# bliunlpr/Robust_e2e_gan

Measured on AMD Instinct MI355X. Metric: joint_train utterances/sec, higher is better.
Workload: dtype f32; 1 GPU; config4: joint_train.py full GAN+ASR step, B=32 per GPU, T=800, F=257->80, L=40, V=4233, enhancer 2xBLSTM-256, VGG+3xBLSTMP-512, loc-attention decoder 300, D basic ndf64, Adadelta; global_batch=32, per_rank_batch=32, parallelism=dp1, utterance_lengths=560..800 frames (mean 680 of T=800)

## Files before the change

### robust_e2e_gan_amd/csrc/lstm.hip

```cpp
#include <stdlib.h>

#include <atomic>

#include "common.h"

namespace {

#ifdef RE2E_EXPERIMENTS
__device__ unsigned long long* g_lstm_stamps = nullptr;
constexpr int kStampStep0 = 64;
#define LSTM_STAMP_DECL unsigned long long* const stamp_p = g_lstm_stamps
#define LSTM_STAMP(ph)                                                                                                              \
  do {                                                                                                                              \
    if (stamp_p && (threadIdx.x & 63) == 0 && s >= kStampStep0 && s < kStampStep0 + 16)                                             \
      stamp_p[((((long)blockIdx.z * gridDim.y + blockIdx.y) * gridDim.x + blockIdx.x) * 16 + (threadIdx.x >> 6)) * 192 + (s - kStampStep0) * 12 + (ph)] = \
          (ph) >= 10 ? __builtin_amdgcn_s_memrealtime() : __builtin_amdgcn_s_memtime();                                             \
  } while (0)
static void lstm_stamps_arm() {
  const char* v = getenv("RE2E_LSTM_STAMPS");
  unsigned long long* p = v ? (unsigned long long*)strtoull(v, nullptr, 16) : nullptr;
  (void)hipMemcpyToSymbol(HIP_SYMBOL(g_lstm_stamps), &p, sizeof(p));
}
#else
#define LSTM_STAMP_DECL
// ... 95 lines not shown
    int idx = tid + it * NTH;
    int bm = idx >> 3, jj = idx & 7, b = b0 + bm, j = j0 + jj;
    if (idx >= 256 || b >= B) continue;
    float v[4];
#pragma unroll
    for (int g = 0; g < 4; ++g) {
      float a = 0.f;
      for (int w = 0; w < WAVES; ++w) a += red[w * (32 * 33) + bm * 33 + g * 8 + jj];
      v[g] = a + pre[it][g];
    }
    float gi = sigmoidf_(v[0]), gf = sigmoidf_(v[1]), gg = tanhf_(v[2]), go = sigmoidf_(v[3]);
    float c = gf * cp[it] + gi * gg;
    float h = go * tanhf_(c);
    if (t >= ln[it]) { c = 0.f; h = 0.f; }
    float* go_ = xg + ((long)t * B + b) * 4 * H + j;
    go_[0] = gi; go_[H] = gf; go_[2 * H] = gg; go_[3 * H] = go;
    cbuf[((long)(t + 1) * B + b) * H2 + dir * H + j] = c;
    ybuf[((long)(t + 1) * B + b) * H2 + dir * H + j] = h;
    hf_wr[((long)(j >> 2) * 32 + bm) * 4 + (j & 3)] = h;
  }
}

typedef unsigned long long u64;
typedef unsigned u32x4 __attribute__((ext_vector_type(4)));
typedef __attribute__((address_space(1))) u64 gu64;
__device__ unsigned g_persist_aborts = 0;
constexpr unsigned kSpinLimit = 1u << 24;

template <int WAVES, int QN, int UW>
__global__ __launch_bounds__(WAVES * 64) void lstm_fwd_persist(float* xg_f, float* xg_r, const float* __restrict__ wfrag, float* ybuf,
                                                               float* cbuf, u64* hx_, unsigned* err, const int* __restrict__ lens,
                                                               int T, int B, int H) {
  extern __shared__ __attribute__((aligned(16))) float red[];
  static_assert(WAVES >= 4 * UW, "256 threads per 8 units own the 32 x 8 cell updates");
  const int dir = blockIdx.z, mt = blockIdx.y, MT = gridDim.y, NX = gridDim.x * UW;
  const int tid = threadIdx.x, lane = tid & 63, wid = tid >> 6, lr = lane & 31, lh = lane >> 5;
  const int usub = (tid >> 8) < UW ? (tid >> 8) : 0;
  const int x = blockIdx.x * UW + usub;
  float* xg = dir ? xg_r : xg_f;
  const int j0 = x * 8, b0 = mt * 32;
  constexpr int kAbort = UW * WAVES * 32 * 33;
  if (tid == 0) red[kAbort] = 0.f;
  const long H2 = 2L * H;
  f32x4 w[UW][QN];
#pragma unroll
  for (int u = 0; u < UW; ++u) {
    const f32x4* wp = reinterpret_cast<const f32x4*>(wfrag) + ((long)(dir * NX + blockIdx.x * UW + u) * NX + wid * QN) * 64 + lane;
#pragma unroll
    for (int q = 0; q < QN; ++q) w[u][q] = wp[q * 64];
  }
  gu64* hx = (gu64*)hx_;
  const int par_sz = 2 * MT * NX * 256;
  const __amdgpu_buffer_rsrc_t hx_rs = __builtin_amdgcn_make_buffer_rsrc(hx_, 0, (int)(2 * par_sz * 8), 0x00020000);
  const int grp = (dir * MT + mt) * NX * 256;
  const int rd_off = grp + (wid * QN) * 256 + (lh * 32 + lr) * 4;
  const bool pw = tid < 256 * UW;
  const int bm = (tid >> 3) & 31, jj = tid & 7, b = b0 + bm, j = j0 + jj;
  const bool ok = pw && b < B;
  const int ln = ok ? lens[b] : 0;
  const int wr_off = grp + x * 256 + ((jj >> 2) * 32 + bm) * 4 + (jj & 3);
  float c = 0.f, pre[4] = {0.f, 0.f, 0.f, 0.f};
  if (ok) {
    const float* gp = xg + ((long)(dir ? T - 1 : 0) * B + b) * 4 * H + j;
#pragma unroll
    for (int g = 0; g < 4; ++g) pre[g] = gp[g * H];
  }
  LSTM_STAMP_DECL;
  __syncthreads();
  for (int s = 0; s < T; ++s) {
    const int t = dir ? T - 1 - s : s;
    LSTM_STAMP(0); LSTM_STAMP(10);
    f32x16 acc[UW];
// ... 1 lines not shown
    for (int u = 0; u < UW; ++u)
#pragma unroll
      for (int r = 0; r < 16; ++r) acc[u][r] = 0.f;
    if (s > 0) {
      const gu64* src = hx + ((s & 1) ^ 1) * par_sz + rd_off;
      float hv[QN][4];
      const unsigned rd_b = (unsigned)((((s & 1) ^ 1) * par_sz + rd_off) * 8);
      for (unsigned spins = 0;; ++spins) {
        asm volatile("" ::: "memory");
        bool good = true;
#pragma unroll
        for (int q = 0; q < QN; ++q) {
          const u32x4 lo = __builtin_amdgcn_raw_buffer_load_b128(hx_rs, rd_b + (unsigned)q * 2048u, 0, 16);
          const u32x4 hi = __builtin_amdgcn_raw_buffer_load_b128(hx_rs, rd_b + (unsigned)q * 2048u + 16u, 0, 16);
          hv[q][0] = __uint_as_float(lo[0]); hv[q][1] = __uint_as_float(lo[2]);
          hv[q][2] = __uint_as_float(hi[0]); hv[q][3] = __uint_as_float(hi[2]);
          good &= (lo[1] == (unsigned)s) & (lo[3] == (unsigned)s) & (hi[1] == (unsigned)s) & (hi[3] == (unsigned)s);
        }
        if (__all(good)) break;
        if (spins > kSpinLimit) { if (lane == 0) { red[kAbort] = 1.f; if (atomicExch(err, 1u) == 0u) atomicAdd(&g_persist_aborts, 1u); } break; }
        __builtin_amdgcn_s_sleep(1);
      }
      LSTM_STAMP(1);
#pragma unroll
      for (int q = 0; q < QN; ++q)
#pragma unroll
        for (int i = 0; i < 4; ++i)
#pragma unroll
          for (int u = 0; u < UW; ++u) acc[u] = __builtin_amdgcn_mfma_f32_32x32x2f32(hv[q][i], w[u][q][i], acc[u], 0, 0, 0);
    }
#pragma unroll
    for (int u = 0; u < UW; ++u) store_acc(red + (u * WAVES + wid) * (32 * 33), acc[u], lane);
    LSTM_STAMP(2);
    __syncthreads();
    LSTM_STAMP(3);
    if (red[kAbort] != 0.f) break;
    if (pw) {
      float v[4];
#pragma unroll
      for (int g = 0; g < 4; ++g) {
        float a = 0.f;
#pragma unroll
        for (int wv = 0; wv < WAVES; ++wv) a += red[(usub * WAVES + wv) * (32 * 33) + bm * 33 + g * 8 + jj];
        v[g] = a + pre[g];
      }
      float gi = sigmoidf_(v[0]), gf = sigmoidf_(v[1]), gg = tanhf_(v[2]), go = sigmoidf_(v[3]);
      float cn = gf * c + gi * gg;
      float h = go * tanhf_(cn);
      if (t >= ln) { cn = 0.f; h = 0.f; }
      c = cn;
      if (ok && s + 1 < T) {
        const float* gp = xg + ((long)(dir ? t - 1 : t + 1) * B + b) * 4 * H + j;
// ... 8 lines not shown
        float* go_ = xg + ((long)t * B + b) * 4 * H + j;
        go_[0] = gi; go_[H] = gf; go_[2 * H] = gg; go_[3 * H] = go;
        cbuf[((long)(t + 1) * B + b) * H2 + dir * H + j] = cn;
        ybuf[((long)(t + 1) * B + b) * H2 + dir * H + j] = h;
      }
    }
    LSTM_STAMP(5);
    __syncthreads();
    LSTM_STAMP(6);
  }
  if (red[kAbort] != 0.f && ok) {
    for (int t = 0; t < T; ++t) ybuf[((long)(t + 1) * B + b) * H2 + dir * H + j] = __uint_as_float(0x7fc00000u);
  }
}

__device__ __forceinline__ void store16u_sc1(unsigned* p, const u32x4& v) {
  asm volatile("global_store_dwordx4 %0, %1, off sc1\n\ts_nop 1" ::"v"(p), "v"(v) : "memory");
}
constexpr unsigned kTagBit = 0x40000000u, kNanPub = 0x3FC00000u;
__device__ __forceinline__ bool tags_are(const u32x4& v, unsigned want) {
  return (((v[0] & v[1] & v[2] & v[3]) ^ want) & kTagBit) == 0u && (((v[0] | v[1] | v[2] | v[3]) ^ want) & kTagBit) == 0u;
}

template <int TILES, int NJ, bool PERSIST>
__global__ __launch_bounds__(256) void lstm_fwd2(float* xg_f, float* xg_r, const float* __restrict__ whh_f, const float* __restrict__ whh_r,
                                                 float* ybuf, float* cbuf, unsigned* hx_, unsigned* err, const int* __restrict__ lens, int T,
                                                 int B, int H, int s_arg) {
  constexpr int KS = 4;
  extern __shared__ __attribute__((aligned(16))) float lds2[];
  f32x4* part = reinterpret_cast<f32x4*>(lds2);
  int* abortw = reinterpret_cast<int*>(lds2 + 2 * TILES * KS * 64 * 4);
  const int dir = blockIdx.z, mt = blockIdx.y, MT = gridDim.y, x = blockIdx.x;
  const int tid = threadIdx.x, lane = tid & 63, ks = tid >> 6, n = lane & 15, kk = lane >> 4;
  const int ft = ks < TILES ? ks : -1;
  float* xg = dir ? xg_r : xg_f;
  const float* whh = dir ? whh_r : whh_f;
  const long H2 = 2L * H;
  if (PERSIST && tid == 0) *abortw = 0;
  f32x4 w[TILES][NJ];
#pragma unroll
  for (int t = 0; t < TILES; ++t) {
    const long row = (long)(n & 3) * H + 4 * TILES * x + 4 * t + (n >> 2);
#pragma unroll
    for (int jj = 0; jj < NJ; ++jj) w[t][jj] = *reinterpret_cast<const f32x4*>(whh + row * H + 16 * (ks * NJ + jj) + 4 * kk);
  }
  const int par_w = 2 * MT * H * 16;
  const __amdgpu_buffer_rsrc_t hx_rs = __builtin_amdgcn_make_buffer_rsrc(hx_, 0, (int)(2 * par_w * 4), 0x00020000);
  const bool fin = ft >= 0;
  const int j = 4 * TILES * x + 4 * (fin ? ft : 0) + kk;
  const int s0 = PERSIST ? 0 : s_arg, s1 = PERSIST ? T : s_arg + 1;
  const int grp = (dir * MT + mt) * H * 16;
  const int b = 16 * mt + n;
  const unsigned rd_w = (unsigned)(grp + ((4 * ks * NJ + kk) * 16 + n) * 4);
  const unsigned poll_w = (unsigned)(grp + ((4 * ks * NJ + (lane < 4 * NJ ? lane : 0)) * 16) * 4);
  const bool ok = fin && b < B;
  const int ln = ok ? lens[b] : 0;
  const unsigned wr_w = (unsigned)(grp + ((TILES * x + (fin ? ft : 0)) * 16 + n) * 4);
  float c = 0.f, pre[4] = {0.f, 0.f, 0.f, 0.f};
  if (ok) {
    const int t0 = dir ? T - 1 - s0 : s0;
    const float* gp = xg + ((long)t0 * B + b) * 4 * H + j;
#pragma unroll
    for (int g = 0; g < 4; ++g) pre[g] = gp[g * H];
    if (!PERSIST) c = cbuf[((long)(dir ? t0 + 2 : t0) * B + b) * H2 + dir * H + j];
  }
  u32x4 ld[NJ];
#pragma unroll
// ... 11 lines not shown
    constexpr int NACC = TILES == 1 ? 2 : TILES;
    f32x4 acc[NACC];
#pragma unroll
    for (int tt = 0; tt < NACC; ++tt) acc[tt] = f32x4{0.f, 0.f, 0.f, 0.f};
    if (s > 0) {
      const unsigned want = PERSIST ? (unsigned)((((s - 1) >> 1) + 1) & 1) << 30 : 0u;
      const unsigned rd_b = (unsigned)((((s & 1) ^ 1) * par_w) * 4) + rd_w * 4u;
      const unsigned pl_b = (unsigned)((((s & 1) ^ 1) * par_w) * 4) + poll_w * 4u;
      auto wait_producers = [&]() {
        for (unsigned spins = 0;; ++spins) {
          asm volatile("" ::: "memory");
          const u32x4 pv = __builtin_amdgcn_raw_buffer_load_b128(hx_rs, pl_b, 0, 16);
          if (__all(tags_are(pv, want))) break;
          if (spins > kSpinLimit) { if (lane == 0) { *abortw = 1; if (atomicExch(err, 1u) == 0u) atomicAdd(&g_persist_aborts, 1u); } break; }
        }
        asm volatile("" ::: "memory");
      };
      if (PERSIST) {
        wait_producers();
#pragma unroll
        for (int jj = 0; jj < NJ; ++jj) ld[jj] = __builtin_amdgcn_raw_buffer_load_b128(hx_rs, rd_b + (unsigned)jj * 1024u, 0, 16);
        LSTM_STAMP(7);
      }
#pragma unroll
      for (int jj = 0; jj < NJ; ++jj) {
        u32x4 v = ld[jj];
        if (PERSIST) {
          if (!__all(tags_are(v, want))) {
            wait_producers();
#pragma unroll
            for (int j2 = jj; j2 < NJ; ++j2) ld[j2] = __builtin_amdgcn_raw_buffer_load_b128(hx_rs, rd_b + (unsigned)j2 * 1024u, 0, 16);
            v = ld[jj];
            for (unsigned spins = 0; !__all(tags_are(v, want)); ++spins) {
              asm volatile("" ::: "memory");
              v = __builtin_amdgcn_raw_buffer_load_b128(hx_rs, rd_b + (unsigned)jj * 1024u, 0, 16);
              if (spins > kSpinLimit) { if (lane == 0) { *abortw = 1; if (atomicExch(err, 1u) == 0u) atomicAdd(&g_persist_aborts, 1u); } break; }
            }
          }
        }
        float hv[4];
#pragma unroll
        for (int i = 0; i < 4; ++i) {
          unsigned uu = PERSIST ? (v[i] & ~kTagBit) : v[i];
          if (PERSIST) uu = uu == kNanPub ? 0x7fc00000u : uu;
          hv[i] = __uint_as_float(uu);
        }
#pragma unroll
        for (int i = 0; i < 4; ++i)
#pragma unroll
          for (int tt = 0; tt < TILES; ++tt) {
            const int a = TILES == 1 ? (i & 1) : tt;
            acc[a] = __builtin_amdgcn_mfma_f32_16x16x4f32(w[tt][jj][i], hv[i], acc[a], 0, 0, 0);
          }
      }
      if (TILES == 1) acc[0] += acc[1];
    }
    LSTM_STAMP(1);
    f32x4* pp = part + (s & 1) * (TILES * KS * 64);
#pragma unroll
    for (int tt = 0; tt < TILES; ++tt)
      if (tt != ft) pp[(tt * KS + ks) * 64 + lane] = acc[tt];
    LSTM_STAMP(2);
    __syncthreads();
    LSTM_STAMP(3);
    if (PERSIST && *abortw) break;
    float og[6] = {0.f, 0.f, 0.f, 0.f, 0.f, 0.f};
    if (fin) {
      f32x4 v = {0.f, 0.f, 0.f, 0.f};
      f32x4 mine = acc[0];
#pragma unroll
      for (int tt = 1; tt < TILES; ++tt) mine = ft == tt ? acc[tt] : mine;
#pragma unroll
      for (int k2 = 0; k2 < KS; ++k2) v += k2 == ks ? mine : pp[(ft * KS + k2) * 64 + lane];
      const float gi = sigmoidf_(v[0] + pre[0]), gf = sigmoidf_(v[1] + pre[1]), gg = tanhf_(v[2] + pre[2]), go = sigmoidf_(v[3] + pre[3]);
      float cn = __builtin_fmaf(gf, c, gi * gg);
      float h = go * tanhf_(cn);
// ... 316 lines not shown
    LSTM_STAMP(8); LSTM_STAMP(11);
    if (lane == 0)
      __hip_atomic_store(flags + (s & 1) * f_par + f_grp + (long)x * 32 + wid * 8, (unsigned)(s + 1), __ATOMIC_RELAXED, __HIP_MEMORY_SCOPE_AGENT);
  }
#pragma unroll
  for (int u = 0; u < UW; ++u) {
    const int j = j0 + 8 * u + jj;
    if (ok) dc_state[(long)b * H2 + dir * H + j] = dcr[u];
    if (aborted && ok) {
      for (int t = 0; t < T; ++t) G[((long)t * B + b) * K4 + j] = __uint_as_float(0x7fc00000u);
    }
  }
}

__global__ void pack_w_bwd3_kernel(const float* __restrict__ whh, float* __restrict__ wb, int H, int UN) {
  const long tot = (long)(H / UN) * (H / 16) * UN * 64;
  for (long e = (long)blockIdx.x * blockDim.x + threadIdx.x; e < tot; e += (long)gridDim.x * blockDim.x) {
    const int lane = (int)(e & 63); long r = e >> 6; const int ks = (int)(r % UN); r /= UN; const int jt = (int)(r % (H / 16)); const int x = (int)(r / (H / 16));
    const int kappa = (lane >> 4) * UN + ks;
    wb[e] = whh[((long)(kappa / UN) * H + (long)x * UN + kappa % UN) * H + 16 * jt + (lane & 15)];
  }
}

template <int UN, int TPW>
__global__ __launch_bounds__(256) void lstm_bwd3(float* g_f, float* g_r, const float* __restrict__ wb, const float* __restrict__ dy,
                                                 const float* __restrict__ cbuf, float* dc_state, float* xbuf, unsigned* flags_, unsigned* err,
                                                 const int* __restrict__ lens, int T, int B, int H, float* __restrict__ dbp) {
  constexpr int KG = 4 * UN;
  constexpr int LDG = KG + 4;
  constexpr int BLK = 16 * UN;
  constexpr int BPI = 1024 / (BLK * 4);
  __shared__ __attribute__((aligned(16))) float dgs[16 * LDG];
  __shared__ __attribute__((aligned(16))) float psum[4 * 256];
  __shared__ int aborted;
  const int dir = blockIdx.z, mt = blockIdx.y, x = blockIdx.x, MT = gridDim.y, NX = gridDim.x;
  float* G = dir ? g_r : g_f;
  const int j0 = x * UN, b0 = mt * 16;
  const int tid = threadIdx.x, lane = tid & 63, wid = tid >> 6, n = lane & 15, kq = lane >> 4;
  const int K4 = 4 * H;
  const long H2 = 2L * H;
  if (tid == 0) aborted = 0;
  float wreg[TPW][UN];
  {
    const float* wp = wb + ((long)(dir * NX + x) * (H / 16)) * UN * 64 + lane;
#pragma unroll
    for (int u = 0; u < TPW; ++u)
#pragma unroll
      for (int ks = 0; ks < UN; ++ks) wreg[u][ks] = wp[((long)(wid + 4 * u) * UN + ks) * 64];
  }
  const long grp = (long)(dir * MT + mt);
  const long x_par = (long)2 * MT * NX * NX * BLK;
  float* xg = xbuf + grp * NX * NX * BLK;
  const __amdgpu_buffer_rsrc_t x_rs = __builtin_amdgcn_make_buffer_rsrc(xbuf, 0, (int)(2 * x_par * 4), 0x00020000);
  gu32* flags = (gu32*)flags_;
  const long f_par = (long)2 * MT * NX * 32;
  const long f_grp = grp * NX * 32;
  const bool cell = tid < 16 * UN;
  const int bm = cell ? tid / UN : 0, jj = tid % UN, b = b0 + bm, j = j0 + jj;
  const bool ok = cell && b < B;
  const long bb = ok ? b : 0;
  const int ln = lens[bb];
  float dcr = 0.f;
  float sbi = 0.f, sbf = 0.f, sbg = 0.f, sbo = 0.f;
  float n_dy, n_g[4], n_c, n_cp;
  {
    const int t = dir ? 0 : T - 1;
    const int prev_blk = dir ? t + 2 : t;
    n_dy = dy[((long)t * B + bb) * H2 + dir * H + j];
    const float* gp0 = G + ((long)t * B + bb) * K4 + j;
#pragma unroll
    for (int g = 0; g < 4; ++g) n_g[g] = gp0[g * H];
// ... 66 lines not shown
      if (cell) {
        const int e = bm * UN + jj;
        if (BPI == 1) dh += (psum[e] + psum[256 + e]) + (psum[512 + e] + psum[768 + e]);
        else dh += ((psum[e] + psum[128 + e]) + (psum[256 + e] + psum[384 + e])) + ((psum[512 + e] + psum[640 + e]) + (psum[768 + e] + psum[896 + e]));
      }
    }
    if (cell) {
      float di = 0.f, df = 0.f, dg = 0.f, dout = 0.f, dcp = dcr;
      if (ok && t < ln) {
        float tc = tanhf_(c);
        float dct = dh * go * (1.f - tc * tc) + dcr;
        dout = dh * tc * go * (1.f - go);
        di = dct * gg * gi * (1.f - gi);
        df = dct * cp * gf * (1.f - gf);
        dg = dct * gi * (1.f - gg * gg);
        dcp = dct * gf;
      }
      dcr = dcp;
      sbi += di; sbf += df; sbg += dg; sbo += dout;
      if (ok) {
        float* gp = G + ((long)t * B + b) * K4 + j;
        gp[0] = di; gp[H] = df; gp[2 * H] = dg; gp[3 * H] = dout;
      }
      float* dq = dgs + bm * LDG + jj;
      dq[0] = di; dq[UN] = df; dq[2 * UN] = dg; dq[3 * UN] = dout;
    }
    LSTM_STAMP(4);
    __syncthreads();
    LSTM_STAMP(5);
    if (s == T - 1) break;
    float bv[UN];
#pragma unroll
    for (int q = 0; q < UN / 4; ++q) {
      const f32x4 t4 = *reinterpret_cast<const f32x4*>(dgs + n * LDG + kq * UN + 4 * q);
      bv[4 * q] = t4[0]; bv[4 * q + 1] = t4[1]; bv[4 * q + 2] = t4[2]; bv[4 * q + 3] = t4[3];
    }
    float* xw = xg + (s & 1) * x_par;
    f32x4 acc[TPW];
    auto store_tile = [&](int u) {
      const int jc0 = 16 * (wid + 4 * u) + 4 * kq;
      float* dst = xw + ((long)(jc0 / UN) * NX + x) * BLK + n * UN + (jc0 % UN);
      store16_sc1(dst, acc[u]);
    };
#pragma unroll
    for (int u0 = 0; u0 < TPW; u0 += 2) {
      acc[u0] = f32x4{0.f, 0.f, 0.f, 0.f};
      if (u0 + 1 < TPW) acc[u0 + 1] = f32x4{0.f, 0.f, 0.f, 0.f};
#pragma unroll
      for (int ks = 0; ks < UN; ++ks) {
        acc[u0] = __builtin_amdgcn_mfma_f32_16x16x4f32(wreg[u0][ks], bv[ks], acc[u0], 0, 0, 0);
        if (u0 + 1 < TPW) acc[u0 + 1] = __builtin_amdgcn_mfma_f32_16x16x4f32(wreg[u0 + 1][ks], bv[ks], acc[u0 + 1], 0, 0, 0);
        if (u0 >= 2 && (ks == 1 || ks == 3)) {
          __builtin_amdgcn_sched_barrier(0);
          store_tile(u0 - 2 + (ks >> 1));
          __builtin_amdgcn_sched_barrier(0);
        }
      }
    }
    if (TPW % 2 == 0) store_tile(TPW - 2);
    store_tile(TPW - 1);
    LSTM_STAMP(6);
    asm volatile("s_waitcnt vmcnt(0)" ::: "memory");
    LSTM_STAMP(7); LSTM_STAMP(8); LSTM_STAMP(11);
    if (lane == 0)
      __hip_atomic_store(flags + (s & 1) * f_par + f_grp + (long)x * 32 + wid * 8, (unsigned)(s + 1), __ATOMIC_RELAXED, __HIP_MEMORY_SCOPE_AGENT);
  }
  if (ok) dc_state[(long)b * H2 + dir * H + j] = dcr;
  if (dbp) {
    __syncthreads();
    if (cell) {
      float* dq = dgs + bm * LDG + jj;
      dq[0] = sbi; dq[UN] = sbf; dq[2 * UN] = sbg; dq[3 * UN] = sbo;
    }
    __syncthreads();
// ... 78 lines not shown
bool is_built(SeqFamily family, int a, int b) {
#define RE2E_HAS(A, B) if (a == A && b == B) return true;
  switch (family) {
    case kFwd2Persist: case kFwd2Step: RE2E_FWD2_ALL(RE2E_HAS) break;
    case kFwdPersist: RE2E_FWD_PERSIST_ALL(RE2E_HAS) break;
    case kFwdStep: RE2E_FWD_STEP_ALL(RE2E_HAS) break;
    case kBwd3: RE2E_BWD3_ALL(RE2E_HAS) break;
    case kBwdPersist: RE2E_BWD_PERSIST_ALL(RE2E_HAS) break;
    case kBwdStep: RE2E_BWD_STEP_ALL(RE2E_HAS) break;
  }
#undef RE2E_HAS
  return false;
}

constexpr size_t kCuLds = 160 * 1024;
constexpr size_t kBwdStaticLds = 16 * 1024;
size_t own_cu_lds(long workgroups, int cus, size_t static_lds, size_t needed) {
  return workgroups <= cus / 2 ? kCuLds - static_lds : needed;
}

bool env_off(const char* name) {
  const char* v = getenv(name);
  return v && atoi(v) == 0;
}

bool plan_fwd(int T, int B, int H, bool weights_16B_aligned, int cus, SeqPlan& p) {
  if (H % 8 != 0) return false;
  const bool persist = !env_off("RE2E_LSTM_PERSIST") && T >= 2;
  if (!env_off("RE2E_LSTM_FWD2") && weights_16B_aligned && H % 64 == 0 && (B <= 16 || H >= 384)) {
    const long per = (long)cdiv(B, 16) * 2;
    int tiles = 0;
    for (int lim : {cus / 2, cus})
      for (int tl = 1; tl <= 4 && !tiles; tl *= 2)
        if ((long)(H / (4 * tl)) * per <= lim) tiles = tl;
    const bool resident = persist && tiles;
    if (!tiles) tiles = 4;
    if (is_built(kFwd2Persist, tiles, H / 64)) {
      p = {resident ? kFwd2Persist : kFwd2Step, tiles, H / 64, dim3(H / (4 * tiles), cdiv(B, 16), 2), (size_t)tiles * 8192 + 16};
      if (resident) p.lds = own_cu_lds((long)p.grid.x * p.grid.y * 2, cus, 0, p.lds);
      return true;
    }
  }
  const dim3 grid(H / 8, cdiv(B, 32), 2);
  if (persist && (long)grid.x * grid.y * 2 <= cus) {
#define RE2E_FIT(W, Q) if ((int)grid.x == W * Q) { p = {kFwdPersist, W, Q, grid, own_cu_lds((long)grid.x * grid.y * 2, cus, 0, (size_t)W * 32 * 33 * sizeof(float) + 16)}; return true; }
    RE2E_FWD_PERSIST_ALL(RE2E_FIT)
// ... 49 lines not shown
  float *wfrag, *hfrag;
  void* hxmem;
  size_t hxbytes;
};
struct BwdArgs {
  float *g_f, *g_r;
  const float *wb, *dy, *cbuf;
  float *dc, *slabs;
  const int* lens;
  int T, B, H;
  void* flagmem;
  size_t flagbytes;
  float* dbp;
};

template <int W>
void launch_fwd_step(const SeqPlan& p, const FwdArgs& a, hipStream_t st) {
  ensure_lds<&lstm_fwd_step<W>>(p.lds);
  const long hn = (long)2 * 2 * p.grid.y * a.H * 32;
  hipLaunchKernelGGL(zero_kernel, dim3(cdiv(hn, 256) > 1024 ? 1024 : cdiv(hn, 256)), dim3(256), 0, st, a.hfrag, hn);
  for (int s = 0; s < a.T; ++s)
    hipLaunchKernelGGL((lstm_fwd_step<W>), p.grid, dim3(W * 64), p.lds, st, a.xg_f, a.xg_r, a.wfrag, a.ybuf, a.cbuf, a.hfrag, a.lens, a.T, a.B, a.H, s);
}
template <int W, int QN>
void launch_fwd_persist(const SeqPlan& p, const FwdArgs& a, hipStream_t st) {
  ensure_lds<&lstm_fwd_persist<W, QN, 1>>(p.lds);
  lstm_stamps_arm();
  (void)hipMemsetAsync(a.hxmem, 0, a.hxbytes, st);
  hipLaunchKernelGGL((lstm_fwd_persist<W, QN, 1>), p.grid, dim3(W * 64), p.lds, st, a.xg_f, a.xg_r, a.wfrag, a.ybuf, a.cbuf, (u64*)((char*)a.hxmem + 16),
                     (unsigned*)a.hxmem, a.lens, a.T, a.B, a.H);
}
template <int TILES, int NJ>
void launch_fwd2_persist(const SeqPlan& p, const FwdArgs& a, hipStream_t st) {
  ensure_lds<&lstm_fwd2<TILES, NJ, true>>(p.lds);
  lstm_stamps_arm();
  (void)hipMemsetAsync(a.hxmem, 0, a.hxbytes, st);
  hipLaunchKernelGGL((lstm_fwd2<TILES, NJ, true>), p.grid, dim3(256), p.lds, st, a.xg_f, a.xg_r, a.whh_f, a.whh_r, a.ybuf, a.cbuf,
                     (unsigned*)((char*)a.hxmem + 16), (unsigned*)a.hxmem, a.lens, a.T, a.B, a.H, 0);
}
template <int TILES, int NJ>
void launch_fwd2_step(const SeqPlan& p, const FwdArgs& a, hipStream_t st) {
  ensure_lds<&lstm_fwd2<TILES, NJ, false>>(p.lds);
  for (int s = 0; s < a.T; ++s)
    hipLaunchKernelGGL((lstm_fwd2<TILES, NJ, false>), p.grid, dim3(256), p.lds, st, a.xg_f, a.xg_r, a.whh_f, a.whh_r, a.ybuf, a.cbuf,
                       (unsigned*)((char*)a.hxmem + 16), (unsigned*)a.hxmem, a.lens, a.T, a.B, a.H, s);
}
template <int JT>
void launch_bwd_step(const SeqPlan& p, const BwdArgs& a, hipStream_t st) {
  for (int s = 0; s < a.T; ++s)
    hipLaunchKernelGGL((lstm_bwd_step<JT>), p.grid, dim3(256), 0, st, a.g_f, a.g_r, a.wb, a.dy, a.cbuf, a.dc, a.slabs, a.lens, a.T, a.B, a.H, s);
}
template <int TPW, int UW>
void launch_bwd_persist(const SeqPlan& p, const BwdArgs& a, hipStream_t st) {
  lstm_stamps_arm();
  (void)hipMemsetAsync(a.flagmem, 0, a.flagbytes, st);
  ensure_lds<&lstm_bwd_persist<TPW, UW>>(p.lds);
  hipLaunchKernelGGL((lstm_bwd_persist<TPW, UW>), p.grid, dim3(256), p.lds, st, a.g_f, a.g_r, a.wb, a.dy, a.cbuf, a.dc, a.slabs,
                     (unsigned*)((char*)a.flagmem + 16), (unsigned*)a.flagmem, a.lens, a.T, a.B, a.H);
}
template <int UN, int TPW>
void launch_bwd3(const SeqPlan& p, const BwdArgs& a, hipStream_t st) {
  lstm_stamps_arm();
  (void)hipMemsetAsync(a.flagmem, 0, a.flagbytes, st);
  ensure_lds<&lstm_bwd3<UN, TPW>>(p.lds);
  hipLaunchKernelGGL((lstm_bwd3<UN, TPW>), p.grid, dim3(256), p.lds, st, a.g_f, a.g_r, a.wb, a.dy, a.cbuf, a.dc, a.slabs,
                     (unsigned*)((char*)a.flagmem + 16), (unsigned*)a.flagmem, a.lens, a.T, a.B, a.H, a.dbp);
}

int run_fwd(const SeqPlan& p, const FwdArgs& args, hipStream_t st) {
  switch (p.family) {
#define RE2E_F2P(A, B) if (p.a == A && p.b == B) return launch_fwd2_persist<A, B>(p, args, st), RE2E_OK;
#define RE2E_F2S(A, B) if (p.a == A && p.b == B) return launch_fwd2_step<A, B>(p, args, st), RE2E_OK;
#define RE2E_FP(A, B) if (p.a == A && p.b == B) return launch_fwd_persist<A, B>(p, args, st), RE2E_OK;
#define RE2E_FS(A, B) if (p.a == A) return launch_fwd_step<A>(p, args, st), RE2E_OK;
    case kFwd2Persist: RE2E_FWD2_ALL(RE2E_F2P) break;
    case kFwd2Step: RE2E_FWD2_ALL(RE2E_F2S) break;
    case kFwdPersist: RE2E_FWD_PERSIST_ALL(RE2E_FP) break;
    case kFwdStep: RE2E_FWD_STEP_ALL(RE2E_FS) break;
    default: break;
#undef RE2E_F2P
#undef RE2E_F2S
#undef RE2E_FP
#undef RE2E_FS
  }
  re2e_set_error("re2e_lstm_seq_fwd: plan %s(%d, %d) is not in the instantiation tables", kFamilyText[p.family].name, p.a, p.b);
  return RE2E_EUNSUPPORTED;
}
int run_bwd(const SeqPlan& p, const BwdArgs& args, hipStream_t st) {
  switch (p.family) {
#define RE2E_B3(A, B) if (p.a == A && p.b == B) return launch_bwd3<A, B>(p, args, st), RE2E_OK;
#define RE2E_BP(A, B) if (p.a == A && p.b == B) return launch_bwd_persist<A, B>(p, args, st), RE2E_OK;
#define RE2E_BS(A, B) if (p.a == A) return launch_bwd_step<A>(p, args, st), RE2E_OK;
    case kBwd3: RE2E_BWD3_ALL(RE2E_B3) break;
    case kBwdPersist: RE2E_BWD_PERSIST_ALL(RE2E_BP) break;
    case kBwdStep: RE2E_BWD_STEP_ALL(RE2E_BS) break;
    default: break;
#undef RE2E_B3
#undef RE2E_BP
#undef RE2E_BS
  }
  re2e_set_error("re2e_lstm_seq_bwd: plan %s(%d, %d) is not in the instantiation tables", kFamilyText[p.family].name, p.a, p.b);
  return RE2E_EUNSUPPORTED;
}

}

namespace {
std::atomic<int> g_force_abort{0};
bool debug_hooks_enabled() {
  static const bool on = [] { const char* e = getenv("RE2E_DEBUG_HOOKS"); return e && atoi(e) == 1; }();
  return on;
}
__global__ void forced_abort_kernel(float* ybuf, long n) {
// ... 17 lines not shown
  if (x < 0.f) sink[0] = occ_lds[0];
}
}

extern "C" int re2e_debug_force_abort(int n) {
  RE2E_CHECK_ARG(n >= 0, "n must be >= 0");
  if (!debug_hooks_enabled()) { re2e_set_error("re2e_debug_force_abort: test hook, needs RE2E_DEBUG_HOOKS=1 in the environment"); return RE2E_EUNSUPPORTED; }
  g_force_abort.store(n, std::memory_order_relaxed);
  return RE2E_OK;
}

extern "C" int re2e_debug_occupy(int workgroups, int lds_bytes, int usec, hipStream_t stream) {
  RE2E_CHECK_ARG(workgroups > 0 && workgroups <= 4096 && lds_bytes >= 1024 && lds_bytes <= 160 * 1024 && usec > 0 && usec <= 1000000, "bad argument");
  if (!debug_hooks_enabled()) { re2e_set_error("re2e_debug_occupy: test hook, needs RE2E_DEBUG_HOOKS=1 in the environment"); return RE2E_EUNSUPPORTED; }
  static LdsLimit lim;
  lim.ensure(reinterpret_cast<const void*>(&occupy_kernel), (size_t)lds_bytes);
  hipLaunchKernelGGL(occupy_kernel, dim3(workgroups), dim3(256), (size_t)lds_bytes, stream, (unsigned long long)usec * 100ull, (float*)nullptr);
  RE2E_LAUNCH_CHECK();
  return RE2E_OK;
}

extern "C" int re2e_warmup(void) {
  const size_t fwd_own = kCuLds, bwd_own = kCuLds - kBwdStaticLds;
#define RE2E_WFP(W, Q) ensure_lds<&lstm_fwd_persist<W, Q, 1>>(fwd_own);
#define RE2E_WF2(TL, NJV) ensure_lds<&lstm_fwd2<TL, NJV, true>>(fwd_own);
#define RE2E_WBP(TP, U) ensure_lds<&lstm_bwd_persist<TP, U>>(bwd_own);
#define RE2E_WB3(U, TP) ensure_lds<&lstm_bwd3<U, TP>>(bwd_own);
  RE2E_FWD_PERSIST_ALL(RE2E_WFP) RE2E_FWD2_ALL(RE2E_WF2) RE2E_BWD_PERSIST_ALL(RE2E_WBP) RE2E_BWD3_ALL(RE2E_WB3)
#undef RE2E_WFP
#undef RE2E_WF2
#undef RE2E_WBP
#undef RE2E_WB3
  hipError_t e = hipGetLastError();
  if (e != hipSuccess) { re2e_set_error("re2e_warmup: %s", hipGetErrorString(e)); return RE2E_EHIP; }
  return RE2E_OK;
}

size_t bwd_dbp_bytes(int B, int H) { return (size_t)2 * ((B + 15) / 16) * 4 * H * sizeof(float); }
extern "C" size_t re2e_lstm_workspace_bytes(int B, int H) {
  size_t a = fwd_ws_floats(B, H) * sizeof(float) + fwd_hx_bytes(B, H), b = bwd_ws_floats(B, H) * sizeof(float) + bwd_flag_bytes(B, H) + bwd_dbp_bytes(B, H);
  return a > b ? a : b;
}

int re2e_dec_abort_count_();

const unsigned* re2e_dec_abort_counter_ptr_();
namespace {
__global__ void step_gate_kernel(const unsigned* dec_cnt, int* base, int ack, const float* extra_sumsq, float* stats_main, float* stats_d,
                                 const float* d_requires, float* hold_next, float* delta_out) {
  const int c = (int)(__hip_atomic_load(&g_persist_aborts, __ATOMIC_RELAXED, __HIP_MEMORY_SCOPE_AGENT) +
// ... 220 lines not shown
```

Baseline: 684.7 utterances/s.

## Emulate fp32 LSTM recurrent matmuls with split-bf16 MFMA (bf16x3)

Splits the recurrent weights and hidden states into three bf16 parts each and accumulates six bf16 MFMA products per k-pair. This replaces the xf32 32x32x2 and 16x16x4 MFMA instructions in the forward persist kernels and the bwd3 backward kernel. The goal is to use the much higher bf16 matrix throughput while keeping near-fp32 accuracy. The cost is extra VALU work to split the hidden state at every step, which is interleaved with the MFMAs through sched_group_barrier hints. It also adds register pressure and an LDS layout change in the backward kernel, and an environment variable restores the fp32 path.

```diff
diff --git a/robust_e2e_gan_amd/csrc/lstm.hip b/robust_e2e_gan_amd/csrc/lstm.hip
--- a/robust_e2e_gan_amd/csrc/lstm.hip
+++ b/robust_e2e_gan_amd/csrc/lstm.hip
@@ -141,12 +141,31 @@
 }
 
 typedef unsigned long long u64;
+typedef __bf16 bf16x8 __attribute__((ext_vector_type(8)));
+__device__ __forceinline__ void split3(float x, __bf16& x1, __bf16& x2, __bf16& x3) {
+  x1 = (__bf16)x;
+  float r = x - (float)x1;
+  x2 = (__bf16)r;
+  r -= (float)x2;
+  x3 = (__bf16)r;
+}
+__device__ __forceinline__ void split3_quad(const f32x4& v, int h, bf16x8 (&pl)[3]) {
+#pragma unroll
+  for (int i = 0; i < 4; ++i) {
+    __bf16 a, b, c;
+    split3(v[i], a, b, c);
+    pl[0][4 * h + i] = a; pl[1][4 * h + i] = b; pl[2][4 * h + i] = c;
+  }
+}
+__host__ __device__ constexpr int split_a(int i) { return i == 0 ? 2 : (i == 1 || i == 3) ? 1 : 0; }
+__host__ __device__ constexpr int split_b(int i) { return i == 2 ? 2 : (i == 1 || i == 4) ? 1 : 0; }
+
 typedef unsigned u32x4 __attribute__((ext_vector_type(4)));
 typedef __attribute__((address_space(1))) u64 gu64;
 __device__ unsigned g_persist_aborts = 0;
 constexpr unsigned kSpinLimit = 1u << 24;
 
-template <int WAVES, int QN, int UW>
+template <int WAVES, int QN, int UW, bool SPLIT>
 __global__ __launch_bounds__(WAVES * 64) void lstm_fwd_persist(float* xg_f, float* xg_r, const float* __restrict__ wfrag, float* ybuf,
                                                                float* cbuf, u64* hx_, unsigned* err, const int* __restrict__ lens,
                                                                int T, int B, int H) {
@@ -161,12 +180,18 @@
   constexpr int kAbort = UW * WAVES * 32 * 33;
   if (tid == 0) red[kAbort] = 0.f;
   const long H2 = 2L * H;
-  f32x4 w[UW][QN];
+  static_assert(!SPLIT || QN % 2 == 0, "a K = 16 instruction takes a pair of k-groups");
+  constexpr int NP = QN / 2;
+  f32x4 w[UW][SPLIT ? 1 : QN];
+  bf16x8 wsp[UW][SPLIT ? NP : 1][3];
 #pragma unroll
   for (int u = 0; u < UW; ++u) {
     const f32x4* wp = reinterpret_cast<const f32x4*>(wfrag) + ((long)(dir * NX + blockIdx.x * UW + u) * NX + wid * QN) * 64 + lane;
 #pragma unroll
-    for (int q = 0; q < QN; ++q) w[u][q] = wp[q * 64];
+    for (int q = 0; q < QN; ++q) {
+      if constexpr (SPLIT) split3_quad(wp[q * 64], q & 1, wsp[u][q >> 1]);
+      else w[u][q] = wp[q * 64];
+    }
   }
   gu64* hx = (gu64*)hx_;
   const int par_sz = 2 * MT * NX * 256;
@@ -214,12 +239,37 @@
         __builtin_amdgcn_s_sleep(1);
       }
       LSTM_STAMP(1);
-#pragma unroll
-      for (int q = 0; q < QN; ++q)
-#pragma unroll
-        for (int i = 0; i < 4; ++i)
-#pragma unroll
-          for (int u = 0; u < UW; ++u) acc[u] = __builtin_amdgcn_mfma_f32_32x32x2f32(hv[q][i], w[u][q][i], acc[u], 0, 0, 0);
+      if constexpr (SPLIT) {
+        bf16x8 hb[2][3];
+        split3_quad(f32x4{hv[0][0], hv[0][1], hv[0][2], hv[0][3]}, 0, hb[0]);
+        split3_quad(f32x4{hv[1][0], hv[1][1], hv[1][2], hv[1][3]}, 1, hb[0]);
+#pragma unroll
+        for (int p = 0; p < NP; ++p) {
+          if (p + 1 < NP) {
+            split3_quad(f32x4{hv[2 * p + 2][0], hv[2 * p + 2][1], hv[2 * p + 2][2], hv[2 * p + 2][3]}, 0, hb[(p + 1) & 1]);
+            split3_quad(f32x4{hv[2 * p + 3][0], hv[2 * p + 3][1], hv[2 * p + 3][2], hv[2 * p + 3][3]}, 1, hb[(p + 1) & 1]);
+          }
+#pragma unroll
+          for (int i = 0; i < 6; ++i)
+#pragma unroll
+            for (int u = 0; u < UW; ++u)
+              acc[u] = __builtin_amdgcn_mfma_f32_32x32x16_bf16(hb[p & 1][split_a(i)], wsp[u][p][split_b(i)], acc[u], 0, 0, 0);
+          if (p + 1 < NP) {
+#pragma unroll
+            for (int i = 0; i < 6 * UW; ++i) {
+              __builtin_amdgcn_sched_group_barrier(0x008, 1, 0);
+              __builtin_amdgcn_sched_group_barrier(0x002, (54 + 6 * UW - 1) / (6 * UW), 0);
+            }
+          }
+        }
+      } else {
+#pragma unroll
+        for (int q = 0; q < QN; ++q)
+#pragma unroll
+          for (int i = 0; i < 4; ++i)
+#pragma unroll
+            for (int u = 0; u < UW; ++u) acc[u] = __builtin_amdgcn_mfma_f32_32x32x2f32(hv[q][i], w[u][q][i], acc[u], 0, 0, 0);
+      }
     }
 #pragma unroll
     for (int u = 0; u < UW; ++u) store_acc(red + (u * WAVES + wid) * (32 * 33), acc[u], lane);
@@ -274,7 +324,7 @@
   return (((v[0] & v[1] & v[2] & v[3]) ^ want) & kTagBit) == 0u && (((v[0] | v[1] | v[2] | v[3]) ^ want) & kTagBit) == 0u;
 }
 
-template <int TILES, int NJ, bool PERSIST>
+template <int TILES, int NJ, bool PERSIST, bool SPLIT>
 __global__ __launch_bounds__(256) void lstm_fwd2(float* xg_f, float* xg_r, const float* __restrict__ whh_f, const float* __restrict__ whh_r,
                                                  float* ybuf, float* cbuf, unsigned* hx_, unsigned* err, const int* __restrict__ lens, int T,
                                                  int B, int H, int s_arg) {
@@ -289,12 +339,19 @@
   const float* whh = dir ? whh_r : whh_f;
   const long H2 = 2L * H;
   if (PERSIST && tid == 0) *abortw = 0;
-  f32x4 w[TILES][NJ];
+  static_assert(!SPLIT || NJ % 2 == 0, "a K = 32 instruction takes a pair of chunks");
+  constexpr int NP = NJ / 2;
+  f32x4 w[SPLIT ? 1 : TILES][SPLIT ? 1 : NJ];
+  bf16x8 ws[SPLIT ? TILES : 1][SPLIT ? NP : 1][3];
 #pragma unroll
   for (int t = 0; t < TILES; ++t) {
     const long row = (long)(n & 3) * H + 4 * TILES * x + 4 * t + (n >> 2);
 #pragma unroll
-    for (int jj = 0; jj < NJ; ++jj) w[t][jj] = *reinterpret_cast<const f32x4*>(whh + row * H + 16 * (ks * NJ + jj) + 4 * kk);
+    for (int jj = 0; jj < NJ; ++jj) {
+      const f32x4 wv = *reinterpret_cast<const f32x4*>(whh + row * H + 16 * (ks * NJ + jj) + 4 * kk);
+      if constexpr (SPLIT) split3_quad(wv, jj & 1, ws[t][jj >> 1]);
+      else w[t][jj] = wv;
+    }
   }
   const int par_w = 2 * MT * H * 16;
   const __amdgpu_buffer_rsrc_t hx_rs = __builtin_amdgcn_make_buffer_rsrc(hx_, 0, (int)(2 * par_w * 4), 0x00020000);
@@ -352,8 +409,7 @@
         for (int jj = 0; jj < NJ; ++jj) ld[jj] = __builtin_amdgcn_raw_buffer_load_b128(hx_rs, rd_b + (unsigned)jj * 1024u, 0, 16);
         LSTM_STAMP(7);
       }
-#pragma unroll
-      for (int jj = 0; jj < NJ; ++jj) {
+      auto chunk = [&](int jj) {
         u32x4 v = ld[jj];
         if (PERSIST) {
           if (!__all(tags_are(v, want))) {
@@ -368,20 +424,57 @@
             }
           }
         }
-        float hv[4];
+        f32x4 hv;
 #pragma unroll
         for (int i = 0; i < 4; ++i) {
           unsigned uu = PERSIST ? (v[i] & ~kTagBit) : v[i];
           if (PERSIST) uu = uu == kNanPub ? 0x7fc00000u : uu;
           hv[i] = __uint_as_float(uu);
         }
-#pragma unroll
-        for (int i = 0; i < 4; ++i)
-#pragma unroll
-          for (int tt = 0; tt < TILES; ++tt) {
-            const int a = TILES == 1 ? (i & 1) : tt;
-            acc[a] = __builtin_amdgcn_mfma_f32_16x16x4f32(w[tt][jj][i], hv[i], acc[a], 0, 0, 0);
+        return hv;
+      };
+      if constexpr (SPLIT) {
+        bf16x8 hb[2][3];
+        {
+          const f32x4 h0 = chunk(0), h1 = chunk(1);
+          split3_quad(h0, 0, hb[0]);
+          split3_quad(h1, 1, hb[0]);
+        }
+#pragma unroll
+        for (int p = 0; p < NP; ++p) {
+          if (p + 1 < NP) {
+            const f32x4 h0 = chunk(2 * p + 2), h1 = chunk(2 * p + 3);
+            split3_quad(h0, 0, hb[(p + 1) & 1]);
+            split3_quad(h1, 1, hb[(p + 1) & 1]);
           }
+#pragma unroll
+          for (int i = 0; i < 6; ++i)
+#pragma unroll
+            for (int tt = 0; tt < TILES; ++tt) {
+              const int a = TILES == 1 ? (i & 1) : tt;
+              acc[a] = __builtin_amdgcn_mfma_f32_16x16x32_bf16(ws[tt][p][split_a(i)], hb[p & 1][split_b(i)], acc[a], 0, 0, 0);
+            }
+          if (p + 1 < NP) {
+            constexpr int kValuPerMfma = (100 + 6 * TILES - 1) / (6 * TILES);
+#pragma unroll
+            for (int i = 0; i < 6 * TILES; ++i) {
+              __builtin_amdgcn_sched_group_barrier(0x008, 1, 0);
+              __builtin_amdgcn_sched_group_barrier(0x002, kValuPerMfma, 0);
+            }
+          }
+        }
+      } else {
+#pragma unroll
+        for (int jj = 0; jj < NJ; ++jj) {
+          const f32x4 hv = chunk(jj);
+#pragma unroll
+          for (int i = 0; i < 4; ++i)
+#pragma unroll
+            for (int tt = 0; tt < TILES; ++tt) {
+              const int a = TILES == 1 ? (i & 1) : tt;
+              acc[a] = __builtin_amdgcn_mfma_f32_16x16x4f32(w[tt][jj][i], hv[i], acc[a], 0, 0, 0);
+            }
+        }
       }
       if (TILES == 1) acc[0] += acc[1];
     }
@@ -744,7 +837,7 @@
   }
 }
 
-template <int UN, int TPW>
+template <int UN, int TPW, bool SPLIT>
 __global__ __launch_bounds__(256) void lstm_bwd3(float* g_f, float* g_r, const float* __restrict__ wb, const float* __restrict__ dy,
                                                  const float* __restrict__ cbuf, float* dc_state, float* xbuf, unsigned* flags_, unsigned* err,
                                                  const int* __restrict__ lens, int T, int B, int H, float* __restrict__ dbp) {
@@ -752,7 +845,10 @@
   constexpr int LDG = KG + 4;
   constexpr int BLK = 16 * UN;
   constexpr int BPI = 1024 / (BLK * 4);
-  __shared__ __attribute__((aligned(16))) float dgs[16 * LDG];
+  constexpr int LDP = KG + 8;
+  constexpr int NH = UN / 8;
+  __shared__ __attribute__((aligned(16))) float dgs[SPLIT && 3 * 16 * LDP / 2 > 16 * LDG ? 3 * 16 * LDP / 2 : 16 * LDG];
+  __bf16* const dgp = reinterpret_cast<__bf16*>(dgs);
   __shared__ __attribute__((aligned(16))) float psum[4 * 256];
   __shared__ int aborted;
   const int dir = blockIdx.z, mt = blockIdx.y, x = blockIdx.x, MT = gridDim.y, NX = gridDim.x;
@@ -762,13 +858,23 @@
   const int K4 = 4 * H;
   const long H2 = 2L * H;
   if (tid == 0) aborted = 0;
-  float wreg[TPW][UN];
+  float wreg[SPLIT ? 1 : TPW][SPLIT ? 1 : UN];
+  bf16x8 wsp[SPLIT ? TPW : 1][SPLIT ? NH : 1][3];
   {
     const float* wp = wb + ((long)(dir * NX + x) * (H / 16)) * UN * 64 + lane;
 #pragma unroll
     for (int u = 0; u < TPW; ++u)
 #pragma unroll
-      for (int ks = 0; ks < UN; ++ks) wreg[u][ks] = wp[((long)(wid + 4 * u) * UN + ks) * 64];
+      for (int ks = 0; ks < UN; ++ks) {
+        const float wv = wp[((long)(wid + 4 * u) * UN + ks) * 64];
+        if constexpr (SPLIT) {
+          __bf16 w1, w2, w3;
+          split3(wv, w1, w2, w3);
+          wsp[u][ks >> 3][0][ks & 7] = w1; wsp[u][ks >> 3][1][ks & 7] = w2; wsp[u][ks >> 3][2][ks & 7] = w3;
+        } else {
+          wreg[u][ks] = wv;
+        }
+      }
   }
   const long grp = (long)(dir * MT + mt);
   const long x_par = (long)2 * MT * NX * NX * BLK;
@@ -881,18 +987,37 @@
         float* gp = G + ((long)t * B + b) * K4 + j;
         gp[0] = di; gp[H] = df; gp[2 * H] = dg; gp[3 * H] = dout;
       }
-      float* dq = dgs + bm * LDG + jj;
-      dq[0] = di; dq[UN] = df; dq[2 * UN] = dg; dq[3 * UN] = dout;
+      if constexpr (SPLIT) {
+        const float dv[4] = {di, df, dg, dout};
+        __bf16* dq = dgp + bm * LDP + jj;
+#pragma unroll
+        for (int g = 0; g < 4; ++g) {
+          __bf16 d1, d2, d3;
+          split3(dv[g], d1, d2, d3);
+          dq[g * UN] = d1; dq[16 * LDP + g * UN] = d2; dq[2 * 16 * LDP + g * UN] = d3;
+        }
+      } else {
+        float* dq = dgs + bm * LDG + jj;
+        dq[0] = di; dq[UN] = df; dq[2 * UN] = dg; dq[3 * UN] = dout;
+      }
     }
     LSTM_STAMP(4);
     __syncthreads();
     LSTM_STAMP(5);
     if (s == T - 1) break;
-    float bv[UN];
-#pragma unroll
-    for (int q = 0; q < UN / 4; ++q) {
-      const f32x4 t4 = *reinterpret_cast<const f32x4*>(dgs + n * LDG + kq * UN + 4 * q);
-      bv[4 * q] = t4[0]; bv[4 * q + 1] = t4[1]; bv[4 * q + 2] = t4[2]; bv[4 * q + 3] = t4[3];
+    float bv[SPLIT ? 1 : UN];
+    bf16x8 bsp[SPLIT ? NH : 1][3];
+    if constexpr (SPLIT) {
+#pragma unroll
+      for (int h = 0; h < NH; ++h)
+#pragma unroll
+        for (int pl = 0; pl < 3; ++pl) bsp[h][pl] = *reinterpret_cast<const bf16x8*>(dgp + (pl * 16 + n) * LDP + kq * UN + 8 * h);
+    } else {
+#pragma unroll
+      for (int q = 0; q < UN / 4; ++q) {
+        const f32x4 t4 = *reinterpret_cast<const f32x4*>(dgs + n * LDG + kq * UN + 4 * q);
+        bv[4 * q] = t4[0]; bv[4 * q + 1] = t4[1]; bv[4 * q + 2] = t4[2]; bv[4 * q + 3] = t4[3];
+      }
     }
     float* xw = xg + (s & 1) * x_par;
     f32x4 acc[TPW];
@@ -906,9 +1031,15 @@
       acc[u0] = f32x4{0.f, 0.f, 0.f, 0.f};
       if (u0 + 1 < TPW) acc[u0 + 1] = f32x4{0.f, 0.f, 0.f, 0.f};
 #pragma unroll
-      for (int ks = 0; ks < UN; ++ks) {
-        acc[u0] = __builtin_amdgcn_mfma_f32_16x16x4f32(wreg[u0][ks], bv[ks], acc[u0], 0, 0, 0);
-        if (u0 + 1 < TPW) acc[u0 + 1] = __builtin_amdgcn_mfma_f32_16x16x4f32(wreg[u0 + 1][ks], bv[ks], acc[u0 + 1], 0, 0, 0);
+      for (int ks = 0; ks < (SPLIT ? 6 * NH : UN); ++ks) {
+        if constexpr (SPLIT) {
+          const int h = ks / 6, r = ks % 6, i = r == 1 ? 2 : r == 2 ? 1 : r;
+          acc[u0] = __builtin_amdgcn_mfma_f32_16x16x32_bf16(wsp[u0][h][split_a(i)], bsp[h][split_b(i)], acc[u0], 0, 0, 0);
+          if (u0 + 1 < TPW) acc[u0 + 1] = __builtin_amdgcn_mfma_f32_16x16x32_bf16(wsp[u0 + 1][h][split_a(i)], bsp[h][split_b(i)], acc[u0 + 1], 0, 0, 0);
+        } else {
+          acc[u0] = __builtin_amdgcn_mfma_f32_16x16x4f32(wreg[u0][ks], bv[ks], acc[u0], 0, 0, 0);
+          if (u0 + 1 < TPW) acc[u0 + 1] = __builtin_amdgcn_mfma_f32_16x16x4f32(wreg[u0 + 1][ks], bv[ks], acc[u0 + 1], 0, 0, 0);
+        }
         if (u0 >= 2 && (ks == 1 || ks == 3)) {
           __builtin_amdgcn_sched_barrier(0);
           store_tile(u0 - 2 + (ks >> 1));
@@ -1033,6 +1164,11 @@
 bool env_off(const char* name) {
   const char* v = getenv(name);
   return v && atoi(v) == 0;
+}
+
+bool fp32_mfma() {
+  const char* v = getenv("RE2E_LSTM_FP32_MFMA");
+  return v && atoi(v) == 1;
 }
 
 bool plan_fwd(int T, int B, int H, bool weights_16B_aligned, int cus, SeqPlan& p) {
@@ -1128,27 +1264,27 @@
   for (int s = 0; s < a.T; ++s)
     hipLaunchKernelGGL((lstm_fwd_step<W>), p.grid, dim3(W * 64), p.lds, st, a.xg_f, a.xg_r, a.wfrag, a.ybuf, a.cbuf, a.hfrag, a.lens, a.T, a.B, a.H, s);
 }
-template <int W, int QN>
+template <int W, int QN, bool SPLIT>
 void launch_fwd_persist(const SeqPlan& p, const FwdArgs& a, hipStream_t st) {
-  ensure_lds<&lstm_fwd_persist<W, QN, 1>>(p.lds);
+  ensure_lds<&lstm_fwd_persist<W, QN, 1, SPLIT>>(p.lds);
   lstm_stamps_arm();
   (void)hipMemsetAsync(a.hxmem, 0, a.hxbytes, st);
-  hipLaunchKernelGGL((lstm_fwd_persist<W, QN, 1>), p.grid, dim3(W * 64), p.lds, st, a.xg_f, a.xg_r, a.wfrag, a.ybuf, a.cbuf, (u64*)((char*)a.hxmem + 16),
+  hipLaunchKernelGGL((lstm_fwd_persist<W, QN, 1, SPLIT>), p.grid, dim3(W * 64), p.lds, st, a.xg_f, a.xg_r, a.wfrag, a.ybuf, a.cbuf, (u64*)((char*)a.hxmem + 16),
                      (unsigned*)a.hxmem, a.lens, a.T, a.B, a.H);
 }
-template <int TILES, int NJ>
+template <int TILES, int NJ, bool SPLIT>
 void launch_fwd2_persist(const SeqPlan& p, const FwdArgs& a, hipStream_t st) {
-  ensure_lds<&lstm_fwd2<TILES, NJ, true>>(p.lds);
+  ensure_lds<&lstm_fwd2<TILES, NJ, true, SPLIT>>(p.lds);
   lstm_stamps_arm();
   (void)hipMemsetAsync(a.hxmem, 0, a.hxbytes, st);
-  hipLaunchKernelGGL((lstm_fwd2<TILES, NJ, true>), p.grid, dim3(256), p.lds, st, a.xg_f, a.xg_r, a.whh_f, a.whh_r, a.ybuf, a.cbuf,
+  hipLaunchKernelGGL((lstm_fwd2<TILES, NJ, true, SPLIT>), p.grid, dim3(256), p.lds, st, a.xg_f, a.xg_r, a.whh_f, a.whh_r, a.ybuf, a.cbuf,
                      (unsigned*)((char*)a.hxmem + 16), (unsigned*)a.hxmem, a.lens, a.T, a.B, a.H, 0);
 }
-template <int TILES, int NJ>
+template <int TILES, int NJ, bool SPLIT>
 void launch_fwd2_step(const SeqPlan& p, const FwdArgs& a, hipStream_t st) {
-  ensure_lds<&lstm_fwd2<TILES, NJ, false>>(p.lds);
+  ensure_lds<&lstm_fwd2<TILES, NJ, false, SPLIT>>(p.lds);
   for (int s = 0; s < a.T; ++s)
-    hipLaunchKernelGGL((lstm_fwd2<TILES, NJ, false>), p.grid, dim3(256), p.lds, st, a.xg_f, a.xg_r, a.whh_f, a.whh_r, a.ybuf, a.cbuf,
+    hipLaunchKernelGGL((lstm_fwd2<TILES, NJ, false, SPLIT>), p.grid, dim3(256), p.lds, st, a.xg_f, a.xg_r, a.whh_f, a.whh_r, a.ybuf, a.cbuf,
                        (unsigned*)((char*)a.hxmem + 16), (unsigned*)a.hxmem, a.lens, a.T, a.B, a.H, s);
 }
 template <int JT>
@@ -1164,20 +1300,21 @@
   hipLaunchKernelGGL((lstm_bwd_persist<TPW, UW>), p.grid, dim3(256), p.lds, st, a.g_f, a.g_r, a.wb, a.dy, a.cbuf, a.dc, a.slabs,
                      (unsigned*)((char*)a.flagmem + 16), (unsigned*)a.flagmem, a.lens, a.T, a.B, a.H);
 }
-template <int UN, int TPW>
+template <int UN, int TPW, bool SPLIT>
 void launch_bwd3(const SeqPlan& p, const BwdArgs& a, hipStream_t st) {
   lstm_stamps_arm();
   (void)hipMemsetAsync(a.flagmem, 0, a.flagbytes, st);
-  ensure_lds<&lstm_bwd3<UN, TPW>>(p.lds);
-  hipLaunchKernelGGL((lstm_bwd3<UN, TPW>), p.grid, dim3(256), p.lds, st, a.g_f, a.g_r, a.wb, a.dy, a.cbuf, a.dc, a.slabs,
+  ensure_lds<&lstm_bwd3<UN, TPW, SPLIT>>(p.lds);
+  hipLaunchKernelGGL((lstm_bwd3<UN, TPW, SPLIT>), p.grid, dim3(256), p.lds, st, a.g_f, a.g_r, a.wb, a.dy, a.cbuf, a.dc, a.slabs,
                      (unsigned*)((char*)a.flagmem + 16), (unsigned*)a.flagmem, a.lens, a.T, a.B, a.H, a.dbp);
 }
 
 int run_fwd(const SeqPlan& p, const FwdArgs& args, hipStream_t st) {
+  const bool fp32 = fp32_mfma();
   switch (p.family) {
-#define RE2E_F2P(A, B) if (p.a == A && p.b == B) return launch_fwd2_persist<A, B>(p, args, st), RE2E_OK;
-#define RE2E_F2S(A, B) if (p.a == A && p.b == B) return launch_fwd2_step<A, B>(p, args, st), RE2E_OK;
-#define RE2E_FP(A, B) if (p.a == A && p.b == B) return launch_fwd_persist<A, B>(p, args, st), RE2E_OK;
+#define RE2E_F2P(A, B) if (p.a == A && p.b == B) return (B % 2 == 0 && !fp32 ? launch_fwd2_persist<A, B, B % 2 == 0> : launch_fwd2_persist<A, B, false>)(p, args, st), RE2E_OK;
+#define RE2E_F2S(A, B) if (p.a == A && p.b == B) return (B % 2 == 0 && !fp32 ? launch_fwd2_step<A, B, B % 2 == 0> : launch_fwd2_step<A, B, false>)(p, args, st), RE2E_OK;
+#define RE2E_FP(A, B) if (p.a == A && p.b == B) return (B % 2 == 0 && !fp32 ? launch_fwd_persist<A, B, B % 2 == 0> : launch_fwd_persist<A, B, false>)(p, args, st), RE2E_OK;
 #define RE2E_FS(A, B) if (p.a == A) return launch_fwd_step<A>(p, args, st), RE2E_OK;
     case kFwd2Persist: RE2E_FWD2_ALL(RE2E_F2P) break;
     case kFwd2Step: RE2E_FWD2_ALL(RE2E_F2S) break;
@@ -1194,7 +1331,7 @@
 }
 int run_bwd(const SeqPlan& p, const BwdArgs& args, hipStream_t st) {
   switch (p.family) {
-#define RE2E_B3(A, B) if (p.a == A && p.b == B) return launch_bwd3<A, B>(p, args, st), RE2E_OK;
+#define RE2E_B3(A, B) if (p.a == A && p.b == B) return (fp32_mfma() ? launch_bwd3<A, B, false> : launch_bwd3<A, B, true>)(p, args, st), RE2E_OK;
 #define RE2E_BP(A, B) if (p.a == A && p.b == B) return launch_bwd_persist<A, B>(p, args, st), RE2E_OK;
 #define RE2E_BS(A, B) if (p.a == A) return launch_bwd_step<A>(p, args, st), RE2E_OK;
     case kBwd3: RE2E_BWD3_ALL(RE2E_B3) break;
@@ -1258,10 +1395,10 @@
 
 extern "C" int re2e_warmup(void) {
   const size_t fwd_own = kCuLds, bwd_own = kCuLds - kBwdStaticLds;
-#define RE2E_WFP(W, Q) ensure_lds<&lstm_fwd_persist<W, Q, 1>>(fwd_own);
-#define RE2E_WF2(TL, NJV) ensure_lds<&lstm_fwd2<TL, NJV, true>>(fwd_own);
+#define RE2E_WFP(W, Q) ensure_lds<&lstm_fwd_persist<W, Q, 1, Q % 2 == 0>>(fwd_own);
+#define RE2E_WF2(TL, NJV) ensure_lds<&lstm_fwd2<TL, NJV, true, NJV % 2 == 0>>(fwd_own);
 #define RE2E_WBP(TP, U) ensure_lds<&lstm_bwd_persist<TP, U>>(bwd_own);
-#define RE2E_WB3(U, TP) ensure_lds<&lstm_bwd3<U, TP>>(bwd_own);
+#define RE2E_WB3(U, TP) ensure_lds<&lstm_bwd3<U, TP, true>>(bwd_own);
   RE2E_FWD_PERSIST_ALL(RE2E_WFP) RE2E_FWD2_ALL(RE2E_WF2) RE2E_BWD_PERSIST_ALL(RE2E_WBP) RE2E_BWD3_ALL(RE2E_WB3)
 #undef RE2E_WFP
 #undef RE2E_WF2
```

Result: no change. 687.2 utterances/s (median of 6 runs) (+0.4%).
